# david-mathews-1994/deltarice

Hardware: AMD Instinct MI355X
Metric: encode+decode GB/s (int16 in) (higher is better)
Workload: dtype int16; 1 GPU; 1000000x7000 int16 Gaussian(sigma=10), m=8, 500 chunks of 2000x7000 per GPU, encode then decode, HBM resident; waveforms_per_gpu=1000000, wave_len=7000, rice_m=8, chunks_per_gpu=500, decode_impl=8

## Files before the change

deltarice_amd/csrc/drx_encode.h:

```cpp
#ifndef DRX_ENCODE_H
#define DRX_ENCODE_H
#include <hip/hip_runtime.h>
#include <stdint.h>

#include "drx_device.h"

namespace drx {

constexpr int kTile = 512;

typedef uint16_t u16x2 __attribute__((ext_vector_type(2)));
typedef int16_t i16x2 __attribute__((ext_vector_type(2)));
__device__ __forceinline__ u16x2 as_u16x2(uint32_t x) { return __builtin_bit_cast(u16x2, x); }
__device__ __forceinline__ i16x2 as_i16x2(uint32_t x) { return __builtin_bit_cast(i16x2, x); }
__device__ __forceinline__ uint32_t as_u32(u16x2 x) { return __builtin_bit_cast(uint32_t, x); }
__device__ __forceinline__ u16x2 splat(uint32_t v) { return (u16x2){(uint16_t)v, (uint16_t)v}; }

struct PackedCodes { uint32_t nb[4], c16[4], e[4]; };

template <bool GEN>
__device__ __forceinline__ void packed_codes(const uint32_t x[4], uint32_t xprev, uint32_t xprev2, const u16x2 (&tp)[4],
                                             uint32_t k, PackedCodes &c) {
    const u16x2 kv = splat(k), kp1 = splat(k + 1u), c16k = splat(16u - k);
    const u16x2 mlo = splat((1u << k) - 1u), mdelta = splat(0xffffu - ((1u << k) - 1u));
    u16x2 z[4], qc[4], e[4];
#pragma unroll
    for (int j = 0; j < 4; ++j) {
        const uint32_t xm1 = j ? x[j - 1] : xprev;
        const uint32_t before = __builtin_amdgcn_alignbit(x[j], xm1, 16);
        i16x2 d;
        if (GEN) {
            const uint32_t xm2 = j >= 2 ? x[j - 2] : (j == 1 ? xprev : xprev2);
            const uint32_t before3 = __builtin_amdgcn_alignbit(xm1, xm2, 16);
            d = __builtin_bit_cast(i16x2, (u16x2)(as_u16x2(x[j]) * tp[0] + as_u16x2(before) * tp[1] +
                                                  as_u16x2(xm1) * tp[2] + as_u16x2(before3) * tp[3]));
        } else {
            d = as_i16x2(x[j]) - as_i16x2(before);
        }
        z[j] = __builtin_bit_cast(u16x2, (i16x2)(d << (int16_t)1)) ^
               __builtin_bit_cast(u16x2, (i16x2)(d >> (int16_t)15));
    }
#pragma unroll
    for (int j = 0; j < 4; ++j) qc[j] = __builtin_elementwise_min((u16x2)(z[j] >> kv), splat(8u));
#pragma unroll
    for (int j = 0; j < 4; ++j) e[j] = qc[j] >> (uint16_t)3;
#pragma unroll
    for (int j = 0; j < 4; ++j) c.nb[j] = as_u32(e[j] * c16k + (qc[j] + kp1));
    const uint32_t mword = as_u32(splat(1u << k));
#pragma unroll
    for (int j = 0; j < 4; ++j) {
        const uint32_t mask = as_u32(e[j] * mdelta + mlo);
        c.c16[j] = (mask & as_u32(z[j])) | (~mask & mword);
        c.e[j] = as_u32(e[j]);
    }
}

constexpr uint32_t kEncCapWords = 2048;

__device__ __forceinline__ int load8_dwords(const int16_t *__restrict__ x, uint32_t len, uint32_t t0, int lane,
                                            bool vec_ok, uint32_t w[4]) {
    const uint32_t i0 = t0 + 8u * (uint32_t)lane;
    const int nv = (i0 >= len) ? 0 : (int)((len - i0) < 8u ? (len - i0) : 8u);
    if (vec_ok && nv == 8) {
        const uint4 q = *reinterpret_cast<const uint4 *>(x + i0);
        w[0] = q.x; w[1] = q.y; w[2] = q.z; w[3] = q.w;
    } else {
#pragma unroll
        for (int j = 0; j < 4; ++j) {
            const uint32_t a = (2 * j < nv) ? (uint32_t)(uint16_t)x[i0 + 2 * j] : 0u;
            const uint32_t b = (2 * j + 1 < nv) ? (uint32_t)(uint16_t)x[i0 + 2 * j + 1] : 0u;
            w[j] = a | (b << 16);
        }
    }
    return nv;
}

__device__ __forceinline__ void mask_tail(PackedCodes &c, int nv) {
#pragma unroll
    for (int j = 0; j < 4; ++j) {
        const uint32_t m = (2 * j + 1 < nv) ? 0xffffffffu : ((2 * j < nv) ? 0x0000ffffu : 0u);
        c.nb[j] &= m;
    }
}

__device__ __forceinline__ uint32_t lane_tile_bits(const PackedCodes &c) {
    const u16x2 s = as_u16x2(c.nb[0]) + as_u16x2(c.nb[1]) + as_u16x2(c.nb[2]) + as_u16x2(c.nb[3]);
    const uint32_t v = as_u32(s);
    return (v & 0xffffu) + (v >> 16);
}

template <bool FULL>
__device__ __forceinline__ void emit_tile(const PackedCodes &c, uint32_t pb) {
    typedef uint32_t __attribute__((address_space(3))) lds_u32;
#pragma unroll
    for (int j = 0; j < 8; ++j) {
        const uint32_t n = (j & 1) ? (c.nb[j >> 1] >> 16) : (c.nb[j >> 1] & 0xffffu);
        uint32_t code32 = __builtin_amdgcn_perm(c.e[j >> 1], c.c16[j >> 1], (j & 1) ? 0x07060302u : 0x05040100u);
        if (!FULL) code32 = n ? code32 : 0u;
        const uint32_t pe = pb + n;
        const uint64_t v = (uint64_t)code32 << (((pb & 32u) - pe) & 63u);
        lds_u32 *w = (lds_u32 *)(uintptr_t)((pb >> 3) & ~3u);
        __hip_atomic_fetch_or(w, (uint32_t)(v >> 32), __ATOMIC_RELAXED, __HIP_MEMORY_SCOPE_WORKGROUP);
        if ((uint32_t)v) __hip_atomic_fetch_or(w + 1, (uint32_t)v, __ATOMIC_RELAXED, __HIP_MEMORY_SCOPE_WORKGROUP);
        pb = pe;
    }
}

__device__ __forceinline__ void concat_codes(const PackedCodes &c, uint32_t (&w)[4]) {
    uint32_t w0 = 0, w1 = 0, w2 = 0, w3 = 0;
#pragma unroll
    for (int j = 0; j < 8; ++j) {
        const uint32_t nbj = c.nb[j >> 1];
        const uint32_t n = (j & 1) ? (nbj >> 16) : nbj;
        const uint32_t code32 = __builtin_amdgcn_perm(c.e[j >> 1], c.c16[j >> 1], (j & 1) ? 0x07060302u : 0x05040100u);
        const uint32_t s = 0u - n;
        if (j >= 3) w3 = __builtin_amdgcn_alignbit(w3, w2, s);
        if (j >= 2) w2 = __builtin_amdgcn_alignbit(w2, w1, s);
        if (j >= 1) w1 = __builtin_amdgcn_alignbit(w1, w0, s);
        w0 = (w0 << (n & 31u)) | code32;
    }
    w[0] = w0; w[1] = w1; w[2] = w2; w[3] = w3;
}

__device__ __forceinline__ void place_words(const uint32_t (&wd)[4], uint32_t pe) {
    typedef uint32_t __attribute__((address_space(3))) lds_u32;
    const uint32_t x0 = __builtin_amdgcn_alignbit(wd[0], 0u, pe);
    const uint32_t x1 = __builtin_amdgcn_alignbit(wd[1], wd[0], pe);
    const uint32_t x2 = __builtin_amdgcn_alignbit(wd[2], wd[1], pe);
    const uint32_t x3 = __builtin_amdgcn_alignbit(wd[3], wd[2], pe);
    const uint32_t x4 = __builtin_amdgcn_alignbit(0u, wd[3], pe);
    lds_u32 *w = (lds_u32 *)(uintptr_t)(((pe >> 3) & ~3u) - 16u);
    __hip_atomic_fetch_or(w + 4, x0, __ATOMIC_RELAXED, __HIP_MEMORY_SCOPE_WORKGROUP);
    __hip_atomic_fetch_or(w + 3, x1, __ATOMIC_RELAXED, __HIP_MEMORY_SCOPE_WORKGROUP);
    __hip_atomic_fetch_or(w + 2, x2, __ATOMIC_RELAXED, __HIP_MEMORY_SCOPE_WORKGROUP);
    if (x3 | x4) {
        __hip_atomic_fetch_or(w + 1, x3, __ATOMIC_RELAXED, __HIP_MEMORY_SCOPE_WORKGROUP);
        if (x4) __hip_atomic_fetch_or(w, x4, __ATOMIC_RELAXED, __HIP_MEMORY_SCOPE_WORKGROUP);
    }
}

constexpr uint32_t kBufFront = 4;

__device__ __forceinline__ void zero_row(uint32_t *row, uint32_t words, int lane) {
    for (int i = lane; i < (int)(words / 4u); i += 64) reinterpret_cast<uint4 *>(row)[i] = make_uint4(0, 0, 0, 0);
}

struct TileCodes {
    PackedCodes c;
    uint32_t cw[4], lane_bits, incl, tile_bits;
};

template <bool GEN, bool FULLT>
__device__ __forceinline__ TileCodes code_tile(const uint32_t (&w)[4], int nv, uint32_t &carry, uint32_t &carry2, const u16x2 (&tp)[4],
                                               uint32_t k) {
    TileCodes t;
    const uint32_t xprev = wave_shr1_carry(w[3], carry);
    carry = (uint32_t)__builtin_amdgcn_readlane((int)w[3], 63);
    uint32_t xprev2 = 0;
    if (GEN) {
        xprev2 = wave_shr1_carry(w[2], carry2);
        carry2 = (uint32_t)__builtin_amdgcn_readlane((int)w[2], 63);
    }
    packed_codes<GEN>(w, xprev, xprev2, tp, k, t.c);
    if (!FULLT) mask_tail(t.c, nv);
    t.lane_bits = lane_tile_bits(t.c);
    if (FULLT) concat_codes(t.c, t.cw);
    t.incl = wave_incl_scan_dpp(t.lane_bits);
    t.tile_bits = (uint32_t)__builtin_amdgcn_readlane((int)t.incl, 63);
    return t;
}

template <bool FULLT, typename At>
__device__ __forceinline__ void put_tile(const TileCodes &t, At &&at) {
    if (FULLT && !__any(t.lane_bits > 128u))
        place_words(t.cw, at(t.incl));
    else
        emit_tile<FULLT>(t.c, at(t.incl - t.lane_bits));
}

template <typename B, typename F>
__device__ __forceinline__ void for_full_tiles(const int16_t *__restrict__ x, uint32_t n_full, int lane, B &&between, F &&full) {
    constexpr int kDepth = 3;
    const uint4 *xv = reinterpret_cast<const uint4 *>(x) + lane;
    uint4 q[kDepth];
    uint32_t t = 0;
#pragma unroll
    for (int u = 0; u < kDepth; ++u) {
        q[u] = make_uint4(0, 0, 0, 0);
        if ((uint32_t)u < n_full) q[u] = xv[64 * (size_t)u];
    }
#pragma unroll 1
    for (; t + 2u * kDepth <= n_full; t += kDepth) {
        between();
#pragma unroll
        for (int u = 0; u < kDepth; ++u) {
            const uint32_t w[4] = {q[u].x, q[u].y, q[u].z, q[u].w};
            full(w);
            q[u] = xv[64 * (size_t)(t + u + kDepth)];
        }
    }
#pragma unroll 1
    for (; t < n_full; t += kDepth) {
        between();
#pragma unroll
        for (int u = 0; u < kDepth; ++u) {
            if (t + (uint32_t)u < n_full) {
                const uint32_t w[4] = {q[u].x, q[u].y, q[u].z, q[u].w};
                full(w);
                if (t + (uint32_t)u + kDepth < n_full) q[u] = xv[64 * (size_t)(t + u + kDepth)];
            }
        }
    }
}

template <bool GEN, bool WINDOW>
__device__ __forceinline__ uint64_t recode_tiles(const int16_t *__restrict__ x, uint32_t len, uint32_t carry, uint32_t carry2,
                                                 const u16x2 (&tp)[4], uint32_t k, int lane, uint32_t *row, uint32_t row_words,
                                                 uint32_t *__restrict__ outp, uint32_t P0, uint32_t skip, uint32_t limit, uint64_t cap) {
    zero_row(row, row_words, lane);
    wave_sync();
    uint32_t *buf = row + kBufFront;
    const uint32_t buf_bits = lds_addr(buf) * 8u;
    auto mine = [&](uint64_t idx) -> bool { return !WINDOW || (idx >= skip && idx < limit && idx < cap); };
    uint64_t P = P0;
    uint32_t wn[4];
    int nvn = load8_dwords(x, len, 0u, lane, true, wn);
    for (uint32_t t0 = 0; t0 < len; t0 += kTile) {
        const uint32_t w[4] = {wn[0], wn[1], wn[2], wn[3]};
        const int nv = nvn;
        if (t0 + kTile < len) nvn = load8_dwords(x, len, t0 + kTile, lane, true, wn);
        const TileCodes t = code_tile<GEN, false>(w, nv, carry, carry2, tp, k);
        const uint64_t wfirst = P >> 5;
        const uint32_t at0 = buf_bits + (uint32_t)(P & 31u);
        put_tile<false>(t, [&](uint32_t bit) -> uint32_t { return at0 + bit; });
        P += t.tile_bits;
        wave_sync();
        const uint32_t nfull = (uint32_t)((P >> 5) - wfirst);
        for (uint32_t i = lane; i < nfull; i += 64) {
            if (mine(wfirst + i)) outp[wfirst + i] = buf[i];
            buf[i] = 0;
        }
        wave_sync();
        if (nfull && lane == 0) { const uint32_t cwd = buf[nfull]; buf[nfull] = 0; buf[0] = cwd; }
        wave_sync();
    }
    if (lane == 0) {
        if ((P & 31u) && mine(P >> 5)) outp[P >> 5] = buf[0];
        buf[0] = 0;
    }
    wave_sync();
    return P;
}

template <bool GEN>
__device__ __forceinline__ uint64_t recode_waveform(const int16_t *__restrict__ x, uint32_t len, const u16x2 (&tp)[4], uint32_t k, int lane,
                                                    uint32_t *row, uint32_t row_words, uint32_t *__restrict__ outp) {
    return recode_tiles<GEN, false>(x, len, 0u, 0u, tp, k, lane, row, row_words, outp, 0u, 0u, 0u, 0ull);
}

template <bool GEN>
__device__ __forceinline__ void history_before(const int16_t *__restrict__ x, uint32_t &carry, uint32_t &carry2) {
    carry = (uint32_t)(uint16_t)x[-1] << 16;
    if (GEN) {
        carry |= (uint32_t)(uint16_t)x[-2];
        carry2 = (uint32_t)(uint16_t)x[-4] | ((uint32_t)(uint16_t)x[-3] << 16);
    }
}

template <bool GEN>
__device__ __forceinline__ void recode_range(const int16_t *__restrict__ xw, uint32_t wf_len, uint32_t s_begin, uint32_t s_end, uint64_t Bp,
                                             uint32_t bits_mine, const u16x2 (&tp)[4], uint32_t k, int lane, uint32_t *row,
                                             uint32_t row_words, uint32_t *__restrict__ payload, uint64_t cap_words) {
    const uint32_t P0 = (uint32_t)(Bp & 31u);
    const uint64_t wbase = Bp >> 5;
    const uint32_t more = wf_len - s_end < 32u ? wf_len - s_end : 32u;
    uint32_t carry = 0, carry2 = 0;
    if (s_begin) history_before<GEN>(xw + s_begin, carry, carry2);
    recode_tiles<GEN, true>(xw + s_begin, s_end - s_begin + more, carry, carry2, tp, k, lane, row, row_words, payload + wbase, P0,
                            P0 ? 1u : 0u, (P0 + bits_mine + 31u) >> 5, cap_words > wbase ? cap_words - wbase : 0ull);
}

}
#endif
```

deltarice_amd/csrc/drx_encode_stream.hip:

```cpp
#include <hip/hip_runtime.h>
#include <stdint.h>

#include <type_traits>

#include "drx_internal.h"
#include "drx_device.h"
#include "drx_encode.h"

namespace drx {

constexpr int kEsWaves = 4;
constexpr uint32_t kEsFront = kBufFront;
constexpr uint32_t kEsBack = 12;
constexpr uint64_t kEsFlag = 1ull << 63;
constexpr uint32_t kEsCtrlWords = 32;
constexpr uint32_t kEsRing = kEsRingWords;
constexpr int kEsPollSleep = 4;

__device__ __forceinline__ uint64_t es_load(const uint64_t *p) {
    return __hip_atomic_load(p, __ATOMIC_RELAXED, __HIP_MEMORY_SCOPE_AGENT);
}
__device__ __forceinline__ void es_store(uint64_t *p, uint64_t v) {
    __hip_atomic_store(p, v, __ATOMIC_RELAXED, __HIP_MEMORY_SCOPE_AGENT);
}

constexpr uint32_t kScPer = 8;

__device__ __forceinline__ void es_scanner(uint64_t total, const uint64_t *__restrict__ size, uint64_t *__restrict__ place,
                                           DevStatus *st) {
    const int lane = lane_id();
    if (threadIdx.x >= 64) return;
    __builtin_amdgcn_s_setprio(3);
    uint64_t pos = 0, base = 0;
    uint32_t idle = 0;
    auto sample = [&](uint64_t (&v)[kScPer], uint64_t at) {
#pragma unroll
        for (int j = 0; j < (int)kScPer; ++j) {
            const uint64_t e = at + 64u * j + (uint32_t)lane;
            v[j] = e < total ? es_load(size + e) : kEsFlag;
        }
    };
    while (pos < total) {
        uint64_t v[kScPer];
        const uint64_t bs = pos;
        sample(v, pos);
        uint64_t run = 0;
        bool open = true, big = false;
#pragma unroll
        for (int j = 0; j < (int)kScPer; ++j) {
            const uint64_t e = bs + 64u * j + (uint32_t)lane;
            const uint64_t m = __ballot(e < pos || (v[j] >> 63) != 0);
            const uint32_t l = (m == ~0ull) ? 64u : (uint32_t)__builtin_ctzll(~m);
            run += open ? l : 0u;
            open = open && l == 64u;
            big = big || __any((v[j] & ~kEsFlag) >= (1ull << 24));
        }
        uint64_t end = bs + run;
        end = end < total ? end : total;
        if (end <= pos) {
            if (++idle > (1u << 22)) {
                if (lane == 0) atomicOr(&st->err, kErrInternal);
                return;
            }
            __builtin_amdgcn_s_sleep(1);
            continue;
        }
        idle = 0;
        uint64_t running = 0;
#pragma unroll
        for (int j = 0; j < (int)kScPer; ++j) {
            if (bs + 64u * j < end) {
                const uint64_t e = bs + 64u * j + (uint32_t)lane;
                const bool in = e >= pos && e < end;
                const uint64_t val = in ? (v[j] & ~kEsFlag) : 0ull;
                uint64_t inc;
                if (!big) {
                    inc = wave_incl_scan_dpp((uint32_t)val);
                } else {
                    inc = val;
#pragma unroll
                    for (int d = 1; d < 64; d <<= 1) {
                        const uint64_t t = __shfl_up(inc, d);
                        if (lane >= d) inc += t;
                    }
                }
                if (in) es_store(place + e, kEsFlag | (base + running + inc - val));
                running += big ? __shfl(inc, 63) : (uint64_t)(uint32_t)__builtin_amdgcn_readlane((int)(uint32_t)inc, 63);
            }
        }
        base += running;
        pos = end;
    }
}

template <int WV>
struct EsShared {
    uint32_t role, arrive, ticket[4];
    uint64_t mine[2][WV];
    uint32_t place_t[2];
};

template <int WV>
__device__ __forceinline__ uint32_t es_rendezvous(EsShared<WV> &shm, uint32_t cyc, int lane, int wv, uint32_t *__restrict__ ctrl,
                                                  uint64_t *__restrict__ size, uint32_t Tprev, uint64_t &off) {
    typedef uint32_t __attribute__((address_space(3))) lds_u32;
    uint32_t arr = 0;
    if (lane == 0) arr = __hip_atomic_fetch_add((lds_u32 *)&shm.arrive, 1u, __ATOMIC_RELAXED, __HIP_MEMORY_SCOPE_WORKGROUP);
    arr = (uint32_t)__builtin_amdgcn_readfirstlane((int)arr);
    if (arr == (uint32_t)WV * cyc) {
        if (lane == 0) shm.ticket[cyc & 3u] = atomicAdd(ctrl + 32, 1u);
    }
    __syncthreads();
    const uint32_t T = rfl(shm.ticket[cyc & 3u]);
    if (cyc) {
        uint64_t sum = 0, before = 0;
#pragma unroll
        for (int i = 0; i < WV; ++i) {
            const uint64_t m = rfl64(shm.mine[(cyc - 1u) & 1u][i]);
            sum += m;
            before += i < wv ? m : 0ull;
        }
        off = before;
        if (wv == 0 && lane == 0) es_store(size + Tprev, kEsFlag | sum);
    }
    return T;
}

template <uint32_t RING>
__device__ __forceinline__ uint32_t es_gap(bool pend, uint32_t startA, uint32_t start, uint32_t behind) {
    if (!pend) return RING - 8u;
    const uint32_t d = startA >= start ? startA - start : startA + RING - start;
    return d > behind ? d - behind : 0u;
}

template <typename InLds, typename Wait, typename Copy>
__device__ __forceinline__ bool es_release(bool must, uint64_t P, InLds &&place_in_lds, Wait &&wait_place, Copy &&copy_out) {
    decltype(wait_place()) pl;
    const bool seen = place_in_lds(pl);
    if (!(seen || must)) return false;
    if (!seen) __builtin_amdgcn_s_setprio(0);
    else if (P < (uint64_t)(4u * kTile * 7u)) __builtin_amdgcn_s_setprio(2);
    else __builtin_amdgcn_s_setprio(1);
    copy_out(seen ? pl : wait_place());
    return true;
}

template <bool FULLT, uint32_t RING>
__device__ __forceinline__ void ring_put(const TileCodes &t, uint32_t *row, uint32_t s0, int lane) {
    constexpr uint32_t kRingBits = RING * 32u;
    uint32_t *ring = row + kEsFront;
    const uint32_t ring_bits0 = lds_addr(ring) * 8u;
    put_tile<FULLT>(t, [&](uint32_t bit) -> uint32_t {
        const uint32_t b = s0 + bit;
        return ring_bits0 + (b >= kRingBits ? b - kRingBits : b);
    });
    if (s0 < kRingBits && s0 + t.tile_bits >= kRingBits) {
        wave_sync();
        if (lane < (int)kEsFront) {
            const uint32_t v = row[lane];
            if (v) { ring[RING - kEsFront + lane] |= v; row[lane] = 0; }
        } else if (lane < (int)(kEsFront + kEsBack)) {
            const uint32_t i = (uint32_t)lane - kEsFront, v = ring[RING + i];
            if (v) { ring[i] |= v; ring[RING + i] = 0; }
        }
        wave_sync();
    }
}

static unsigned es_grid(const Geom &G, uint64_t tickets) {
    const unsigned full = 256u * (16u / kEsWaves);
    return (G.dbg & DRX_DBG_STREAM_THREE_WGS) ? 3u : (unsigned)(tickets + 1 < full ? tickets + 1 : full);
}

template <bool GEN, int WV, uint32_t RING>
__global__ __launch_bounds__(64 * WV, 4) void k_encode_stream(Geom G, const int16_t *__restrict__ in, uint32_t *__restrict__ out,
                                                              uint64_t out_cap, uint64_t *__restrict__ chunk_word_off,
                                                              uint32_t *__restrict__ wave_words, uint64_t *__restrict__ size,
                                                              uint64_t *__restrict__ place, uint32_t *__restrict__ ctrl,
                                                              DevStatus *st) {
    __shared__ __attribute__((aligned(16))) uint32_t ring_all[WV][kEsFront + RING + kEsBack];
    __shared__ EsShared<WV> shm;
    __shared__ uint64_t s_place_v[2];
    typedef uint32_t __attribute__((address_space(3))) lds_u32;
    typedef uint64_t __attribute__((address_space(3))) lds_u64;
    static_assert((kEsFront + RING + kEsBack) % 4 == 0 && RING % 4 == 0, "16-byte LDS accesses");
    constexpr uint32_t kRowWords = kEsFront + RING + kEsBack;
    const int lane = lane_id(), wv = wave_id();
    uint32_t *row = ring_all[wv];
    uint32_t *ring = row + kEsFront;

    if (threadIdx.x == 0) {
        shm.role = atomicAdd(ctrl, 1u);
        shm.arrive = 0;
        shm.place_t[0] = shm.place_t[1] = 0;
    }
    zero_row(row, kRowWords, lane);
    __syncthreads();
    const uint64_t n_tickets = (G.total_waves + WV - 1) / WV;
    if (rfl(shm.role) == 0) {
        es_scanner(n_tickets, size, place, st);
        return;
    }

    const uint32_t k = G.k;
    const u16x2 tp[4] = {splat(GEN ? G.enc_t[0] : 1u), splat(GEN ? G.enc_t[1] : 0xffffu), splat(GEN ? G.enc_t[2] : 0u),
                         splat(GEN ? G.enc_t[3] : 0u)};

    bool pend = false, fitsA = true;
    uint64_t gA = 0, offA = 0;
    uint32_t TA = 0, startA = 0, nA = 0;
    WaveRef rA = {};

    auto place_header = [&](const WaveRef &r, uint64_t g, uint32_t n, uint64_t ex, uint64_t &pos) -> bool {
        const uint64_t mine = 1ull + n + (r.idx == 0 ? 1ull : 0ull);
        pos = ex + (r.idx == 0 ? 1ull : 0ull);
        if (lane == 0) {
            if (r.idx == 0) chunk_word_off[r.chunk] = ex;
            if (g + 1 == G.total_waves) {
                chunk_word_off[G.n_chunks] = ex + mine;
                st->total_words = ex + mine;
                if (G.host_words) *G.host_words = ex + mine;
                if (ex + mine > out_cap) atomicOr(&st->err, kErrCapacity);
            }
        }
        const bool room = pos + 1u + n <= out_cap;
        if (room && lane == 0) {
            out[pos] = n;
            if (r.idx == 0) out[pos - 1] = r.n_samples;
        }
        return room;
    };
    auto copy_out = [&](uint64_t ex) {
        uint64_t pos;
        const bool room = place_header(rA, gA, nA, ex + offA, pos);
        uint32_t *__restrict__ outp = out + pos + 1;
        typedef uint32_t u32x4s __attribute__((ext_vector_type(4)));
        typedef u32x4s __attribute__((address_space(1), aligned(4))) g_u32x4_a4;
        const uint32_t n4 = nA & ~3u;
        for (uint32_t i = 4u * (uint32_t)lane; i < n4; i += 256u) {
            uint32_t w = startA + i;
            w = w >= RING ? w - RING : w;
            const uint4 v = *reinterpret_cast<const uint4 *>(ring + w);
            if (room) *(g_u32x4_a4 *)(outp + i) = (u32x4s){v.x, v.y, v.z, v.w};
            *reinterpret_cast<uint4 *>(ring + w) = make_uint4(0, 0, 0, 0);
        }
        if ((uint32_t)lane < nA - n4) {
            uint32_t w = startA + n4 + (uint32_t)lane;
            w = w >= RING ? w - RING : w;
            if (room) outp[n4 + (uint32_t)lane] = ring[w];
            ring[w] = 0;
        }
        wave_sync();
        pend = false;
    };
    auto place_in_lds = [&](uint64_t &ex) -> bool {
        const uint32_t t = __hip_atomic_load((lds_u32 *)&shm.place_t[TA & 1u], __ATOMIC_RELAXED, __HIP_MEMORY_SCOPE_WORKGROUP);
        if (rfl(t) != TA + 1u) return false;
        ex = rfl64(__hip_atomic_load((lds_u64 *)&s_place_v[TA & 1u], __ATOMIC_RELAXED, __HIP_MEMORY_SCOPE_WORKGROUP));
        return true;
    };
    auto place_to_lds = [&](uint64_t ex) {
        if (lane == 0) {
            __hip_atomic_store((lds_u64 *)&s_place_v[TA & 1u], ex, __ATOMIC_RELAXED, __HIP_MEMORY_SCOPE_WORKGROUP);
            __hip_atomic_store((lds_u32 *)&shm.place_t[TA & 1u], TA + 1u, __ATOMIC_RELAXED, __HIP_MEMORY_SCOPE_WORKGROUP);
        }
    };
    auto wait_place = [&]() -> uint64_t {
        uint32_t spins = 0;
        for (;;) {
            uint64_t ex;
            bool have = place_in_lds(ex);
            if (!have) {
                uint64_t v = 0;
                if (lane == 0) v = es_load(place + TA);
                const uint32_t hi = (uint32_t)__builtin_amdgcn_readfirstlane((int)(uint32_t)(v >> 32));
                if (hi >> 31) {
                    ex = ((uint64_t)(hi & 0x7fffffffu) << 32) | (uint32_t)__builtin_amdgcn_readfirstlane((int)(uint32_t)v);
                    place_to_lds(ex);
                    have = true;
                }
            }
            if (have) return ex;
            __builtin_amdgcn_s_sleep(kEsPollSleep);
            if (++spins > (1u << 22)) {
                if (lane == 0) atomicOr(&st->err, kErrInternal);
                return out_cap;
            }
        }
    };

    auto stream_out = [&](uint64_t ex) {
        uint64_t pos;
        const bool room = place_header(rA, gA, nA, ex + offA, pos);
        recode_waveform<GEN>(in + rA.sample_off, room ? rA.len : 0u, tp, k, lane, row, kRowWords, out + pos + 1);
        pend = false;
    };

    uint32_t start = 0;
    uint32_t Tprev = 0;
    for (uint32_t cyc = 0;; ++cyc) {
        const uint32_t T = es_rendezvous(shm, cyc, lane, wv, ctrl, size, Tprev, offA);
        if (pend && !fitsA) stream_out(wait_place());
        if ((uint64_t)T * WV >= G.total_waves) break;
        Tprev = T;
        const uint64_t g = (uint64_t)T * WV + (uint32_t)wv;
        if (g >= G.total_waves) {
            if (lane == 0) shm.mine[cyc & 1u][wv] = 0;
            if (pend) copy_out(wait_place());
            continue;
        }

        const WaveRef r = locate_uniform(G, g);
        const int16_t *x = in + r.sample_off;
        const uint32_t wlen = r.len;

        auto gap = [&]() -> uint32_t { return es_gap<RING>(pend, startA, start, 8u); };
        if (pend && gap() < 512u) copy_out(wait_place());
        uint32_t limit = gap();

        uint64_t P = 0;
        bool fits = true;
        uint32_t carry = 0;
        uint32_t carry2 = 0;
        auto process_tile = [&](const uint32_t (&w)[4], int nv, auto full_tag) {
            constexpr bool FULLT = decltype(full_tag)::value;
            const TileCodes t = code_tile<GEN, FULLT>(w, nv, carry, carry2, tp, k);
            const uint32_t need = ((uint32_t)P + t.tile_bits + 31u) >> 5;
            bool ok = fits && need < limit;
            if (pend && es_release(fits && !ok, P, place_in_lds, wait_place, copy_out)) {
                limit = gap();
                ok = fits && need < limit;
            }
            if (ok)
                ring_put<FULLT, RING>(t, row, start * 32u + (uint32_t)P, lane);
            else
                fits = false;
            P += t.tile_bits;
        };
        const uint32_t n_full = wlen / kTile;
        uint64_t pollv = 0;
        bool polling = false;
        auto between = [&]() {
            if (!pend) return;
            if (polling) {
                const uint32_t hi = (uint32_t)__builtin_amdgcn_readfirstlane((int)(uint32_t)(pollv >> 32));
                polling = false;
                if (hi >> 31) {
                    place_to_lds(((uint64_t)(hi & 0x7fffffffu) << 32) | (uint32_t)__builtin_amdgcn_readfirstlane((int)(uint32_t)pollv));
                    return;
                }
            }
            if (lane == 0) pollv = es_load(place + TA);
            polling = true;
        };

        for_full_tiles(x, n_full, lane, between, [&](const uint32_t (&w)[4]) { process_tile(w, 8, std::true_type{}); });
        for (uint32_t t0 = n_full * kTile; t0 < wlen; t0 += kTile) {
            uint32_t w[4];
            const int nv = load8_dwords(x, wlen, t0, lane, true, w);
            process_tile(w, nv, std::false_type{});
        }
        const uint32_t n = (uint32_t)((P + 31u) >> 5);
        wave_sync();
        if (lane == 0) {
            wave_words[g] = n;
            shm.mine[cyc & 1u][wv] = 1ull + n + (r.idx == 0 ? 1ull : 0ull);
        }
        if (pend) copy_out(wait_place());
        pend = true;
        fitsA = fits;
        gA = g;
        rA = r;
        TA = T;
        startA = start;
        nA = n;
        if (fits) {
            start += (n + 3u) & ~3u;
            start = start >= RING ? start - RING : start;
        }
    }
    if (pend) copy_out(wait_place());
}

struct EsPlace2 { uint64_t whdr, bits; };

__device__ __forceinline__ void es_scanner_segs(uint64_t total, uint32_t tpw, uint32_t waves_per_chunk, const uint64_t *__restrict__ size,
                                                uint64_t *__restrict__ place, DevStatus *st) {
    const int lane = lane_id();
    if (threadIdx.x >= 64) return;
    __builtin_amdgcn_s_setprio(3);
    uint64_t pos = 0;
    uint64_t whdr = 1;
    uint64_t bits_in = 0;
    uint32_t idle = 0;
    const double rcp_tpw = 1.0 / (double)tpw;
    while (pos < total) {
        uint64_t v[kScPer];
        const uint64_t bs = pos;
#pragma unroll
        for (int j = 0; j < (int)kScPer; ++j) {
            const uint64_t e = bs + 64u * j + (uint32_t)lane;
            v[j] = e < total ? es_load(size + e) : 0ull;
        }
        uint64_t run = 0;
        bool open = true;
#pragma unroll
        for (int j = 0; j < (int)kScPer; ++j) {
            const uint64_t m = __ballot((v[j] >> 63) != 0);
            const uint32_t l = (m == ~0ull) ? 64u : (uint32_t)__builtin_ctzll(~m);
            run += open ? l : 0u;
            open = open && l == 64u;
        }
        const uint64_t end = bs + run;
        if (end <= pos) {
            if (++idle > (1u << 22)) {
                if (lane == 0) atomicOr(&st->err, kErrInternal);
                return;
            }
            __builtin_amdgcn_s_sleep(1);
            continue;
        }
        idle = 0;
#pragma unroll
        for (int j = 0; j < (int)kScPer; ++j) {
            if (bs + 64u * j < end) {
                const uint64_t e = bs + 64u * j + (uint32_t)lane;
                const bool in = e < end;
                const uint32_t val = in ? (uint32_t)(v[j] & 0xffffffffull) : 0u;
                const uint32_t e32 = (uint32_t)e;
                uint32_t g = (uint32_t)((double)e32 * rcp_tpw);
                uint32_t jj = e32 - g * tpw;
                if ((int32_t)jj < 0) { g -= 1u; jj += tpw; }
                if (jj >= tpw) { g += 1u; jj -= tpw; }
                const bool closing = in && jj + 1u == tpw;
                const uint32_t inc = wave_incl_scan_dpp(val), ex = inc - val;
                const int f = lane - (int)jj;
                const uint32_t exf = (uint32_t)__shfl((int)ex, f < 0 ? 0 : f);
                const uint64_t before = f < 0 ? bits_in + ex : (uint64_t)(ex - exf);
                const uint64_t nw = closing ? (before + val + 31ull) >> 5 : 0ull;
                const uint64_t contrib = closing ? 1ull + nw + (((g + 1u) % waves_per_chunk == 0u) ? 1ull : 0ull) : 0ull;
                uint64_t cinc;
                if (!__any(contrib >= (1ull << 24))) {
                    cinc = wave_incl_scan_dpp((uint32_t)contrib);
                } else {
                    cinc = contrib;
#pragma unroll
                    for (int d = 1; d < 64; d <<= 1) {
                        const uint64_t t = __shfl_up(cinc, d);
                        if (lane >= d) cinc += t;
                    }
                }
                const uint64_t my_whdr = whdr + cinc - contrib;
                if (in) {
                    es_store(place + 2u * e, kEsFlag | my_whdr);
                    es_store(place + 2u * e + 1u, kEsFlag | before);
                }
                const uint64_t left = end - (bs + 64u * j);
                const int li = __builtin_amdgcn_readfirstlane(left >= 64u ? 63 : (int)left - 1);
                const uint64_t wn = my_whdr + contrib, bn = closing ? 0ull : before + val;
                whdr = ((uint64_t)(uint32_t)__builtin_amdgcn_readlane((int)(uint32_t)(wn >> 32), li) << 32) | (uint32_t)__builtin_amdgcn_readlane((int)(uint32_t)wn, li);
                bits_in = ((uint64_t)(uint32_t)__builtin_amdgcn_readlane((int)(uint32_t)(bn >> 32), li) << 32) | (uint32_t)__builtin_amdgcn_readlane((int)(uint32_t)bn, li);
            }
        }
        pos = end;
    }
}

template <bool GEN, int WV, uint32_t RING>
__global__ __launch_bounds__(64 * WV, 4) void k_encode_stream_segs(Geom G, uint32_t seg_len, uint32_t tpw, const int16_t *__restrict__ in,
                                                                   uint32_t *__restrict__ out, uint64_t out_cap,
                                                                   uint64_t *__restrict__ chunk_word_off, uint32_t *__restrict__ wave_words,
                                                                   uint64_t *__restrict__ size, uint64_t *__restrict__ place,
                                                                   uint32_t *__restrict__ ctrl, DevStatus *st) {
    __shared__ __attribute__((aligned(16))) uint32_t ring_all[WV][kEsFront + RING + kEsBack];
    __shared__ EsShared<WV> shm;
    __shared__ uint64_t s_place_v[2][2];
    __shared__ uint32_t s_first[2][WV];
    typedef uint32_t __attribute__((address_space(3))) lds_u32;
    typedef uint64_t __attribute__((address_space(3))) lds_u64;
    static_assert((kEsFront + RING + kEsBack) % 4 == 0 && RING % 4 == 0, "16-byte LDS accesses");
    static_assert(WV == (int)kEsSegWaves, "es_seg_shape() counts tickets of kEsSegWaves segments");
    constexpr uint32_t kRowWords = kEsFront + RING + kEsBack;
    const int lane = lane_id(), wv = wave_id();
    uint32_t *row = ring_all[wv];
    uint32_t *ring = row + kEsFront;

    if (threadIdx.x == 0) {
        shm.role = atomicAdd(ctrl, 1u);
        shm.arrive = 0;
        shm.place_t[0] = shm.place_t[1] = 0;
    }
    zero_row(row, kRowWords, lane);
    __syncthreads();
    const uint64_t n_tickets = G.total_waves * tpw;
    if (rfl(shm.role) == 0) {
        es_scanner_segs(n_tickets, tpw, G.u_n_waves, size, place, st);
        return;
    }
    const uint32_t k = G.k;
    const u16x2 tp[4] = {splat(GEN ? G.enc_t[0] : 1u), splat(GEN ? G.enc_t[1] : 0xffffu), splat(GEN ? G.enc_t[2] : 0u),
                         splat(GEN ? G.enc_t[3] : 0u)};

    bool pend = false, fitsA = true, lastA = false, sibA = false;
    uint64_t gA = 0, offA = 0;
    uint32_t TA = 0, startA = 0, nA = 0, bitsA = 0, sbeginA = 0, sendA = 0, parA = 0;
    WaveRef rA = {};

    auto headers = [&](const WaveRef &r, const EsPlace2 &pl, uint64_t B) {
        if (lane != 0) return;
        if (sbeginA == 0u && r.idx == 0u) {
            chunk_word_off[r.chunk] = pl.whdr - 1u;
            if (pl.whdr - 1u < out_cap) out[pl.whdr - 1u] = r.n_samples;
        }
        if (lastA) {
            const uint64_t n = (B + bitsA + 31ull) >> 5;
            wave_words[gA] = (uint32_t)n;
            if (pl.whdr < out_cap) out[pl.whdr] = (uint32_t)n;
            if (gA + 1u == G.total_waves) {
                const uint64_t tot = pl.whdr + 1ull + n;
                chunk_word_off[G.n_chunks] = tot;
                st->total_words = tot;
                if (G.host_words) *G.host_words = tot;
                if (tot > out_cap) atomicOr(&st->err, kErrCapacity);
            }
        }
    };
    auto copy_out = [&](const EsPlace2 &pl) {
        const uint64_t B = pl.bits + offA;
        headers(rA, pl, B);
        const uint64_t w0 = pl.whdr + 1ull + (B >> 5);
        const uint32_t s = (uint32_t)B & 31u;
        const uint32_t i_lo = s ? 1u : 0u, i_hi = (s + bitsA + 31u) >> 5;
        const uint32_t nA4 = (nA + 3u) & ~3u, top = nA4 > i_hi ? nA4 : ((i_hi + 3u) & ~3u);
        if (sibA) {
            if (lane == 0) {
                const uint32_t F = s_first[parA][wv + 1], sh = bitsA & 31u;
                uint32_t wi = startA + (bitsA >> 5);
                wi = wi >= RING ? wi - RING : wi;
                ring[wi] |= F >> sh;
                if (sh) {
                    wi = wi + 1u >= RING ? wi + 1u - RING : wi + 1u;
                    ring[wi] |= F << (32u - sh);
                }
            }
            wave_sync();
        }
        uint32_t *__restrict__ outp = out + w0;
        const uint64_t room = out_cap > w0 ? out_cap - w0 : 0ull;
        typedef uint32_t u32x4s __attribute__((ext_vector_type(4)));
        typedef u32x4s __attribute__((address_space(1), aligned(4))) g_u32x4_a4;
        uint32_t carryw = 0;
        for (uint32_t i0 = 0; i0 < top; i0 += 256u) {
            const uint32_t i = i0 + 4u * (uint32_t)lane;
            uint4 v = make_uint4(0, 0, 0, 0);
            uint32_t w = startA + i;
            w = w >= RING ? w - RING : w;
            const bool inr = i < nA4;
            if (inr) v = *reinterpret_cast<const uint4 *>(ring + w);
            uint32_t pw = (uint32_t)__builtin_amdgcn_update_dpp(0, (int)v.w, 0x138, 0xf, 0xf, false);
            if (lane == 0) pw = carryw;
            carryw = (uint32_t)__builtin_amdgcn_readlane((int)v.w, 63);
            const uint32_t o0 = __builtin_amdgcn_alignbit(pw, v.x, s), o1 = __builtin_amdgcn_alignbit(v.x, v.y, s);
            const uint32_t o2 = __builtin_amdgcn_alignbit(v.y, v.z, s), o3 = __builtin_amdgcn_alignbit(v.z, v.w, s);
            if (i >= i_lo && i + 4u <= i_hi && (uint64_t)i + 4u <= room) {
                *(g_u32x4_a4 *)(outp + i) = (u32x4s){o0, o1, o2, o3};
            } else {
                if (i >= i_lo && i < i_hi && (uint64_t)i < room) outp[i] = o0;
                if (i + 1u >= i_lo && i + 1u < i_hi && (uint64_t)i + 1u < room) outp[i + 1u] = o1;
                if (i + 2u >= i_lo && i + 2u < i_hi && (uint64_t)i + 2u < room) outp[i + 2u] = o2;
                if (i + 3u >= i_lo && i + 3u < i_hi && (uint64_t)i + 3u < room) outp[i + 3u] = o3;
            }
            if (inr) *reinterpret_cast<uint4 *>(ring + w) = make_uint4(0, 0, 0, 0);
        }
        wave_sync();
        pend = false;
    };
    auto place_in_lds = [&](EsPlace2 &pl) -> bool {
        const uint32_t t = __hip_atomic_load((lds_u32 *)&shm.place_t[TA & 1u], __ATOMIC_RELAXED, __HIP_MEMORY_SCOPE_WORKGROUP);
        if (rfl(t) != TA + 1u) return false;
        pl.whdr = rfl64(__hip_atomic_load((lds_u64 *)&s_place_v[TA & 1u][0], __ATOMIC_RELAXED, __HIP_MEMORY_SCOPE_WORKGROUP));
        pl.bits = rfl64(__hip_atomic_load((lds_u64 *)&s_place_v[TA & 1u][1], __ATOMIC_RELAXED, __HIP_MEMORY_SCOPE_WORKGROUP));
        return true;
    };
    auto place_to_lds = [&](const EsPlace2 &pl) {
        if (lane == 0) {
            __hip_atomic_store((lds_u64 *)&s_place_v[TA & 1u][0], pl.whdr, __ATOMIC_RELAXED, __HIP_MEMORY_SCOPE_WORKGROUP);
            __hip_atomic_store((lds_u64 *)&s_place_v[TA & 1u][1], pl.bits, __ATOMIC_RELAXED, __HIP_MEMORY_SCOPE_WORKGROUP);
            __hip_atomic_store((lds_u32 *)&shm.place_t[TA & 1u], TA + 1u, __ATOMIC_RELAXED, __HIP_MEMORY_SCOPE_WORKGROUP);
        }
    };
    auto place_of = [&](uint64_t pv, EsPlace2 &pl) -> bool {
        const uint32_t lo = (uint32_t)pv, hi = (uint32_t)(pv >> 32);
        const uint32_t h0 = (uint32_t)__builtin_amdgcn_readlane((int)hi, 0), h1 = (uint32_t)__builtin_amdgcn_readlane((int)hi, 1);
        if (!((h0 & h1) >> 31)) return false;
        pl.whdr = ((uint64_t)(h0 & 0x7fffffffu) << 32) | (uint32_t)__builtin_amdgcn_readlane((int)lo, 0);
        pl.bits = ((uint64_t)(h1 & 0x7fffffffu) << 32) | (uint32_t)__builtin_amdgcn_readlane((int)lo, 1);
        return true;
    };
    auto wait_place = [&]() -> EsPlace2 {
        uint32_t spins = 0;
        for (;;) {
            EsPlace2 pl;
            if (place_in_lds(pl)) return pl;
            uint64_t pv = 0;
            if (lane < 2) pv = es_load(place + 2ull * TA + (uint32_t)lane);
            if (place_of(pv, pl)) {
                place_to_lds(pl);
                return pl;
            }
            __builtin_amdgcn_s_sleep(kEsPollSleep);
            if (++spins > (1u << 22)) {
                if (lane == 0) atomicOr(&st->err, kErrInternal);
                pl.whdr = out_cap;
                pl.bits = 0;
                return pl;
            }
        }
    };

    auto stream_out = [&](const EsPlace2 &pl) {
        const uint64_t B = pl.bits + offA;
        headers(rA, pl, B);
        recode_range<GEN>(in + rA.sample_off, rA.len, sbeginA, sendA, B, bitsA, tp, k, lane, row, kRowWords, out + pl.whdr + 1ull,
                          out_cap > pl.whdr + 1ull ? out_cap - pl.whdr - 1ull : 0ull);
        pend = false;
    };

    uint32_t start = 0;
    uint32_t Tprev = 0;
    for (uint32_t cyc = 0;; ++cyc) {
        const uint32_t T = es_rendezvous(shm, cyc, lane, wv, ctrl, size, Tprev, offA);
        if (pend && !fitsA) stream_out(wait_place());
        if ((uint64_t)T >= n_tickets) break;
        Tprev = T;
        const uint32_t gw = T / tpw, tj = T - gw * tpw;
        const uint64_t g = gw;
        const WaveRef r = locate_uniform(G, g);
        const uint32_t wlen = r.len;
        const uint32_t sgi = tj * (uint32_t)WV + (uint32_t)wv;
        const uint64_t sb64 = (uint64_t)sgi * seg_len;
        if (sb64 >= wlen) {
            if (lane == 0) shm.mine[cyc & 1u][wv] = 0;
            if (pend) copy_out(wait_place());
            continue;
        }
        const uint32_t s_begin = (uint32_t)sb64;
        const uint32_t s_end = wlen - s_begin > seg_len ? s_begin + seg_len : wlen;
        const bool sib = wv + 1 < WV && seg_len >= 32u && wlen - s_end >= 32u;
        const uint32_t more = sib ? 0u : (wlen - s_end < 32u ? wlen - s_end : 32u);
        const uint32_t slen = s_end - s_begin;
        const uint32_t clen = slen + more;
        const int16_t *x = in + r.sample_off + s_begin;

        auto gap = [&]() -> uint32_t { return es_gap<RING>(pend, startA, start, 12u); };
        if (pend && gap() < 512u) copy_out(wait_place());
        uint32_t limit = gap();

        uint64_t P = 0;
        uint32_t seg_bits = 0;
        bool first = true;
        bool fits = true;
        uint32_t carry = 0, carry2 = 0;
        if (s_begin) history_before<GEN>(x, carry, carry2);
        auto process_tile = [&](const uint32_t (&w)[4], int nv, int mark, auto full_tag) {
            constexpr bool FULLT = decltype(full_tag)::value;
            const TileCodes t = code_tile<GEN, FULLT>(w, nv, carry, carry2, tp, k);
            if (!FULLT && mark >= 0) seg_bits = (uint32_t)P + (mark ? (uint32_t)__builtin_amdgcn_readlane((int)t.incl, mark - 1) : 0u);
            const uint32_t need = ((uint32_t)P + t.tile_bits + 31u) >> 5;
            bool ok = fits && need < limit;
            if (pend && es_release(fits && !ok, P, place_in_lds, wait_place, copy_out)) {
                limit = gap();
                ok = fits && need < limit;
            }
            if (ok)
                ring_put<FULLT, RING>(t, row, start * 32u + (uint32_t)P, lane);
            else
                fits = false;
            P += t.tile_bits;
            if (first) {
                first = false;
                wave_sync();
                if (lane == 0) s_first[cyc & 1u][wv] = ring[start];
            }
        };
        const uint32_t n_fast = more ? slen / kTile : clen / kTile;
        uint64_t pollv = 0;
        bool polling = false;
        auto between = [&]() {
            if (!pend) return;
            if (polling) {
                polling = false;
                EsPlace2 pl;
                if (place_of(pollv, pl)) {
                    place_to_lds(pl);
                    return;
                }
            }
            pollv = 0;
            if (lane < 2) pollv = es_load(place + 2ull * TA + (uint32_t)lane);
            polling = true;
        };
        for_full_tiles(x, n_fast, lane, between, [&](const uint32_t (&w)[4]) { process_tile(w, 8, -1, std::true_type{}); });
        for (uint32_t t0 = n_fast * kTile; t0 < clen; t0 += kTile) {
            uint32_t w[4];
            const int nv = load8_dwords(x, clen, t0, lane, true, w);
            const int mark = (more && slen >= t0 && slen < t0 + (uint32_t)kTile) ? (int)((slen - t0) >> 3) : -1;
            process_tile(w, nv, mark, std::false_type{});
        }
        if (!more) seg_bits = (uint32_t)P;
        const uint32_t n = (uint32_t)((P + (sib ? 63u : 31u)) >> 5);
        wave_sync();
        if (lane == 0) shm.mine[cyc & 1u][wv] = seg_bits;
        if (pend) copy_out(wait_place());
        pend = true;
        fitsA = fits;
        gA = g;
        rA = r;
        TA = T;
        startA = start;
        nA = fits ? n : 0u;
        bitsA = seg_bits;
        sbeginA = s_begin;
        sendA = s_end;
        lastA = s_end == wlen;
        sibA = sib;
        parA = cyc & 1u;
        if (fits) {
            start += (n + 3u) & ~3u;
            start = start >= RING ? start - RING : start;
        }
    }
    if (pend) copy_out(wait_place());
}

hipError_t launch_encode_stream(const Geom &G, const int16_t *d_in, uint32_t *d_out, uint64_t out_cap,
                                uint64_t *d_chunk_word_off, uint32_t *d_wave_words, uint64_t *d_scan,
                                DevStatus *d_status, hipEvent_t *ev, hipStream_t s) {
    if (G.total_waves == 0) return hipSuccess;
    const uint64_t W = G.total_waves;
    const uint64_t tickets = (W + kEsWaves - 1) / kEsWaves;
    mark(ev, 0, s);
    hipError_t e = hipMemsetAsync(d_scan, 0, (2 * tickets + kEsCtrlWords) * sizeof(uint64_t), s);
    if (e != hipSuccess) return e;
    mark(ev, 1, s);
    mark(ev, 2, s);
    uint64_t *size = d_scan, *place = d_scan + tickets;
    uint32_t *ctrl = reinterpret_cast<uint32_t *>(d_scan + 2 * tickets);
    const unsigned grid = es_grid(G, tickets);
    if (G.n_taps)
        k_encode_stream<true, kEsWaves, kEsRing><<<grid, 64 * kEsWaves, 0, s>>>(G, d_in, d_out, out_cap, d_chunk_word_off, d_wave_words, size,
                                                                              place, ctrl, d_status);
    else
        k_encode_stream<false, kEsWaves, kEsRing><<<grid, 64 * kEsWaves, 0, s>>>(G, d_in, d_out, out_cap, d_chunk_word_off, d_wave_words, size,
                                                                               place, ctrl, d_status);
    mark(ev, 3, s);
    return hipGetLastError();
}

hipError_t launch_encode_stream_segs(const Geom &G, uint32_t seg_target, const int16_t *d_in, uint32_t *d_out, uint64_t out_cap,
                                     uint64_t *d_chunk_word_off, uint32_t *d_wave_words, uint64_t *d_scan,
                                     DevStatus *d_status, hipEvent_t *ev, hipStream_t s) {
    if (G.total_waves == 0) return hipSuccess;
    const EsSegShape sh = es_seg_shape(G.u_wave_len, seg_target);
    const uint64_t tickets = G.total_waves * sh.tpw;
    mark(ev, 0, s);
    hipError_t e = hipMemsetAsync(d_scan, 0, (3 * tickets + kEsCtrlWords) * sizeof(uint64_t), s);
    if (e != hipSuccess) return e;
    mark(ev, 1, s);
    mark(ev, 2, s);
    uint64_t *size = d_scan, *place = d_scan + tickets;
    uint32_t *ctrl = reinterpret_cast<uint32_t *>(d_scan + 3 * tickets);
    const unsigned grid = es_grid(G, tickets);
    if (G.n_taps)
        k_encode_stream_segs<true, kEsWaves, kEsRing><<<grid, 64 * kEsWaves, 0, s>>>(G, sh.seg_len, sh.tpw, d_in, d_out, out_cap, d_chunk_word_off,
                                                                                   d_wave_words, size, place, ctrl, d_status);
    else
        k_encode_stream_segs<false, kEsWaves, kEsRing><<<grid, 64 * kEsWaves, 0, s>>>(G, sh.seg_len, sh.tpw, d_in, d_out, out_cap, d_chunk_word_off,
                                                                                    d_wave_words, size, place, ctrl, d_status);
    mark(ev, 3, s);
    return hipGetLastError();
}

}
```

Measured before the change: 1531 GB/s.

## Fold tail tile into prefetched tile loop with clamped loads and fast tail packing

Replaces the separate full-tile prefetch loop and the per-tile tail loader with one loop that prefetches through the tail tile using clamped addresses. The tail tile comes from the prefetched registers. Ragged lanes are patched with scalar loads, and codes are concatenated and shifted so the tail can use the fast word-placement path instead of per-code emission. For wave_len=7000 there is a 344-sample tail in every waveform, so this aims to hide the tail's load latency and cut its emission cost. It adds selects, shifts and a manual waitcnt, and changes the loop bounds (n_full vs 2*kDepth), which raises the risk of boundary bugs.

Result: faster. 1577 GB/s (median of 6 runs) (+3.0%).

```diff
diff --git a/deltarice_amd/csrc/drx_encode.h b/deltarice_amd/csrc/drx_encode.h
--- a/deltarice_amd/csrc/drx_encode.h
+++ b/deltarice_amd/csrc/drx_encode.h
@@ -178,6 +178,59 @@
         emit_tile<FULLT>(t.c, at(t.incl - t.lane_bits));
 }
 
+__device__ __forceinline__ void shr128(uint32_t (&w)[4], uint32_t n) {
+    const uint32_t ws = n >> 5;
+    const uint32_t y0 = ws == 0u ? w[0] : ws == 1u ? w[1] : ws == 2u ? w[2] : ws == 3u ? w[3] : 0u;
+    const uint32_t y1 = ws == 0u ? w[1] : ws == 1u ? w[2] : ws == 2u ? w[3] : 0u;
+    const uint32_t y2 = ws == 0u ? w[2] : ws == 1u ? w[3] : 0u;
+    const uint32_t y3 = ws == 0u ? w[3] : 0u;
+    w[0] = __builtin_amdgcn_alignbit(y1, y0, n);
+    w[1] = __builtin_amdgcn_alignbit(y2, y1, n);
+    w[2] = __builtin_amdgcn_alignbit(y3, y2, n);
+    w[3] = y3 >> (n & 31u);
+}
+
+template <bool GEN>
+__device__ __forceinline__ TileCodes code_tail_tile(const uint32_t (&w)[4], int nv, bool ragged, uint32_t &carry, uint32_t &carry2,
+                                                    const u16x2 (&tp)[4], uint32_t k, bool &wide) {
+    TileCodes t;
+    const uint32_t xprev = wave_shr1_carry(w[3], carry);
+    carry = (uint32_t)__builtin_amdgcn_readlane((int)w[3], 63);
+    uint32_t xprev2 = 0;
+    if (GEN) {
+        xprev2 = wave_shr1_carry(w[2], carry2);
+        carry2 = (uint32_t)__builtin_amdgcn_readlane((int)w[2], 63);
+    }
+    packed_codes<GEN>(w, xprev, xprev2, tp, k, t.c);
+    const uint32_t all_bits = lane_tile_bits(t.c);
+    concat_codes(t.c, t.cw);
+    if (ragged) {
+        PackedCodes cm = t.c;
+        mask_tail(cm, nv);
+        t.lane_bits = lane_tile_bits(cm);
+        shr128(t.cw, all_bits - t.lane_bits);
+    } else {
+        t.lane_bits = nv ? all_bits : 0u;
+#pragma unroll
+        for (int j = 0; j < 4; ++j) t.cw[j] = nv ? t.cw[j] : 0u;
+    }
+    wide = __any((nv ? all_bits : 0u) > 128u);
+    t.incl = wave_incl_scan_dpp(t.lane_bits);
+    t.tile_bits = (uint32_t)__builtin_amdgcn_readlane((int)t.incl, 63);
+    return t;
+}
+
+template <typename At>
+__device__ __forceinline__ void put_tail_tile(const TileCodes &t, int nv, bool wide, At &&at) {
+    if (!wide) {
+        place_words(t.cw, at(t.incl));
+    } else {
+        PackedCodes c = t.c;
+        mask_tail(c, nv);
+        emit_tile<false>(c, at(t.incl - t.lane_bits));
+    }
+}
+
 template <typename B, typename F>
 __device__ __forceinline__ void for_full_tiles(const int16_t *__restrict__ x, uint32_t n_full, int lane, B &&between, F &&full) {
     constexpr int kDepth = 3;
@@ -210,6 +263,56 @@
                 if (t + (uint32_t)u + kDepth < n_full) q[u] = xv[64 * (size_t)(t + u + kDepth)];
             }
         }
+    }
+}
+
+template <typename B, typename F, typename T>
+__device__ __forceinline__ void for_tiles(const int16_t *__restrict__ x, uint32_t len, uint32_t n_full, bool tail, int lane,
+                                          B &&between, F &&full, T &&tailf) {
+    constexpr int kDepth = 3;
+    const uint32_t last = tail ? n_full : n_full - 1u;
+    const uint32_t imax = len - 8u;
+    auto load = [&](uint32_t tile) -> uint4 {
+        tile = tile < last ? tile : last;
+        uint32_t i = tile * (uint32_t)kTile + 8u * (uint32_t)lane;
+        i = i < imax ? i : imax;
+        return *reinterpret_cast<const uint4 *>(x + i);
+    };
+    uint4 q[kDepth];
+#pragma unroll
+    for (int u = 0; u < kDepth; ++u) {
+        q[u] = load((uint32_t)u);
+        __builtin_amdgcn_sched_barrier(0);
+    }
+    uint32_t t = 0;
+#pragma unroll 1
+    for (; t + kDepth <= n_full; t += kDepth) {
+        between(true);
+#pragma unroll
+        for (int u = 0; u < kDepth; ++u) {
+            const uint32_t w[4] = {q[u].x, q[u].y, q[u].z, q[u].w};
+            full(w);
+            q[u] = load(t + (uint32_t)u + kDepth);
+        }
+    }
+    const uint32_t left = n_full - t;
+    static_assert(kDepth == 3, "the straight code below");
+    if (left) {
+        between(false);
+        const uint32_t w0[4] = {q[0].x, q[0].y, q[0].z, q[0].w};
+        full(w0);
+        if (left > 1u) {
+            const uint32_t w1[4] = {q[1].x, q[1].y, q[1].z, q[1].w};
+            full(w1);
+        }
+    }
+    if (tail) {
+        auto sel = [left](uint32_t a, uint32_t b, uint32_t c) -> uint32_t { return left == 0u ? a : (left == 1u ? b : c); };
+        const uint32_t w[4] = {sel(q[0].x, q[1].x, q[2].x), sel(q[0].y, q[1].y, q[2].y), sel(q[0].z, q[1].z, q[2].z),
+                               sel(q[0].w, q[1].w, q[2].w)};
+        tailf(w);
+    } else {
+        __builtin_amdgcn_s_waitcnt(0x0f70);
     }
 }
 
diff --git a/deltarice_amd/csrc/drx_encode_stream.hip b/deltarice_amd/csrc/drx_encode_stream.hip
--- a/deltarice_amd/csrc/drx_encode_stream.hip
+++ b/deltarice_amd/csrc/drx_encode_stream.hip
@@ -145,12 +145,12 @@
     return true;
 }
 
-template <bool FULLT, uint32_t RING>
-__device__ __forceinline__ void ring_put(const TileCodes &t, uint32_t *row, uint32_t s0, int lane) {
+template <uint32_t RING, typename Put>
+__device__ __forceinline__ void ring_put_with(const TileCodes &t, uint32_t *row, uint32_t s0, int lane, Put &&put) {
     constexpr uint32_t kRingBits = RING * 32u;
     uint32_t *ring = row + kEsFront;
     const uint32_t ring_bits0 = lds_addr(ring) * 8u;
-    put_tile<FULLT>(t, [&](uint32_t bit) -> uint32_t {
+    put([&](uint32_t bit) -> uint32_t {
         const uint32_t b = s0 + bit;
         return ring_bits0 + (b >= kRingBits ? b - kRingBits : b);
     });
@@ -165,6 +165,10 @@
         }
         wave_sync();
     }
+}
+template <bool FULLT, uint32_t RING>
+__device__ __forceinline__ void ring_put(const TileCodes &t, uint32_t *row, uint32_t s0, int lane) {
+    ring_put_with<RING>(t, row, s0, lane, [&](auto &&at) { put_tile<FULLT>(t, at); });
 }
 
 static unsigned es_grid(const Geom &G, uint64_t tickets) {
@@ -313,6 +317,9 @@
         const WaveRef r = locate_uniform(G, g);
         const int16_t *x = in + r.sample_off;
         const uint32_t wlen = r.len;
+        const uint32_t n_full = wlen / kTile, rem = wlen - n_full * (uint32_t)kTile;
+        const bool tail = rem != 0u, ragged = (rem & 7u) != 0u;
+        const bool tail_lane = 8u * (uint32_t)lane + 8u <= rem;
 
         auto gap = [&]() -> uint32_t { return es_gap<RING>(pend, startA, start, 8u); };
         if (pend && gap() < 512u) copy_out(wait_place());
@@ -324,23 +331,27 @@
         uint32_t carry2 = 0;
         auto process_tile = [&](const uint32_t (&w)[4], int nv, auto full_tag) {
             constexpr bool FULLT = decltype(full_tag)::value;
-            const TileCodes t = code_tile<GEN, FULLT>(w, nv, carry, carry2, tp, k);
+            bool wide = false;
+            TileCodes t;
+            if constexpr (FULLT) t = code_tile<GEN, true>(w, nv, carry, carry2, tp, k);
+            else t = code_tail_tile<GEN>(w, nv, ragged, carry, carry2, tp, k, wide);
             const uint32_t need = ((uint32_t)P + t.tile_bits + 31u) >> 5;
             bool ok = fits && need < limit;
             if (pend && es_release(fits && !ok, P, place_in_lds, wait_place, copy_out)) {
                 limit = gap();
                 ok = fits && need < limit;
             }
-            if (ok)
-                ring_put<FULLT, RING>(t, row, start * 32u + (uint32_t)P, lane);
-            else
+            if (ok) {
+                if constexpr (FULLT) ring_put<true, RING>(t, row, start * 32u + (uint32_t)P, lane);
+                else ring_put_with<RING>(t, row, start * 32u + (uint32_t)P, lane, [&](auto &&at) { put_tail_tile(t, nv, wide, at); });
+            } else {
                 fits = false;
+            }
             P += t.tile_bits;
         };
-        const uint32_t n_full = wlen / kTile;
         uint64_t pollv = 0;
         bool polling = false;
-        auto between = [&]() {
+        auto between = [&](bool again) {
             if (!pend) return;
             if (polling) {
                 const uint32_t hi = (uint32_t)__builtin_amdgcn_readfirstlane((int)(uint32_t)(pollv >> 32));
@@ -350,15 +361,34 @@
                     return;
                 }
             }
+            if (!again) return;
             if (lane == 0) pollv = es_load(place + TA);
             polling = true;
         };
 
-        for_full_tiles(x, n_full, lane, between, [&](const uint32_t (&w)[4]) { process_tile(w, 8, std::true_type{}); });
-        for (uint32_t t0 = n_full * kTile; t0 < wlen; t0 += kTile) {
+        auto full_tile = [&](const uint32_t (&w)[4]) { process_tile(w, 8, std::true_type{}); };
+        auto tail_tile = [&](const uint32_t (&wq)[4]) {
+            const uint32_t i0 = 8u * (uint32_t)lane;
+            const int nv = tail_lane ? 8 : (i0 < rem ? (int)(rem - i0) : 0);
             uint32_t w[4];
-            const int nv = load8_dwords(x, wlen, t0, lane, true, w);
+#pragma unroll
+            for (int j = 0; j < 4; ++j) w[j] = tail_lane ? wq[j] : 0u;
+            if (ragged && nv > 0 && nv < 8) {
+                const int16_t *xl = x + (size_t)n_full * kTile + i0;
+#pragma unroll
+                for (int j = 0; j < 4; ++j) {
+                    const uint32_t a = (2 * j < nv) ? (uint32_t)(uint16_t)xl[2 * j] : 0u;
+                    const uint32_t b = (2 * j + 1 < nv) ? (uint32_t)(uint16_t)xl[2 * j + 1] : 0u;
+                    w[j] = a | (b << 16);
+                }
+            }
             process_tile(w, nv, std::false_type{});
+        };
+        if (wlen >= 8u) {
+            for_tiles(x, wlen, n_full, tail, lane, between, full_tile, tail_tile);
+        } else {
+            const uint32_t none[4] = {0u, 0u, 0u, 0u};
+            tail_tile(none);
         }
         const uint32_t n = (uint32_t)((P + 31u) >> 5);
         wave_sync();
```
